# ShenhanQian/GaussianAvatars

Measured on NVIDIA H100. Metric: rasterizer fwd+bwd frames/sec @100k splats 1080p, higher is better.
Workload: dtype f32

## Files before the change

### gaussianavatars_b200/_native.py

```python
from __future__ import annotations

import ctypes as C
import os
import threading

import torch

_HERE = os.path.dirname(os.path.abspath(__file__))
LIB_PATH = os.path.join(_HERE, "libgaussianavatars_b200.so")

ABI_VERSION = 3
INPUT_ACTIVATED = 0
INPUT_BOUND_RAW = 1
SYNC_EXACT, SYNC_LATE, SYNC_NONE = 0, 1, 2
CTR_NOT_MIN_DEPTH_KEY, CTR_MAX_DEPTH_KEY, CTR_NUM_RENDERED, CTR_NUM_LISTED, CTR_BUCKET_OVERFLOW, CTR_CAPACITY, CTR_SEQ = range(7)
NUM_COUNTERS = 8
TUNE_HEAVY_FWD, TUNE_HEAVY_BWD, TUNE_DEPTH_SORT, TUNE_TILE_SORT, TUNE_NVLS_CTAS = 0, 1, 2, 4, 5

ALLOC_FN = C.CFUNCTYPE(C.c_void_p, C.c_void_p, C.c_size_t)


class ForwardArgs(C.Structure):
    _fields_ = [
        ("abi_version", C.c_uint32), ("input_mode", C.c_int32), ("P", C.c_int32), ("sh_degree", C.c_int32),
        ("sh_coeffs", C.c_int32), ("image_width", C.c_int32), ("image_height", C.c_int32),
        ("tanfovx", C.c_float), ("tanfovy", C.c_float), ("scale_modifier", C.c_float),
        ("prefiltered", C.c_int32), ("debug", C.c_int32), ("need_backward", C.c_int32), ("binning_hint", C.c_int32),
        ("exact_binning", C.c_int32), ("depth_hint_lo", C.c_uint32), ("depth_hint_hi", C.c_uint32),
        ("sync_mode", C.c_int32), ("frame_seq", C.c_uint32), ("counters_host", C.c_void_p),
        ("overflow_flag", C.c_void_p),
        ("bg", C.c_void_p), ("viewmatrix", C.c_void_p), ("projmatrix", C.c_void_p), ("campos", C.c_void_p),
        ("means3D", C.c_void_p), ("opacities", C.c_void_p), ("scales", C.c_void_p), ("rotations", C.c_void_p),
        ("cov3D_precomp", C.c_void_p), ("shs", C.c_void_p), ("sh_dc", C.c_void_p), ("sh_rest", C.c_void_p),
        ("colors_precomp", C.c_void_p),
        ("binding", C.c_void_p), ("num_faces", C.c_int32), ("face_center", C.c_void_p),
        ("face_orien_mat", C.c_void_p), ("face_scaling", C.c_void_p),
        ("out_color", C.c_void_p), ("radii", C.c_void_p), ("visibility", C.c_void_p),
        ("alloc_geom", ALLOC_FN), ("alloc_binning", ALLOC_FN), ("alloc_image", ALLOC_FN), ("alloc_user", C.c_void_p),
    ]


class FrameState(C.Structure):
    _fields_ = [
        ("num_rendered", C.c_int64), ("num_candidates", C.c_int64),
        ("geom_buffer", C.c_void_p), ("binning_buffer", C.c_void_p), ("image_buffer", C.c_void_p),
        ("geom_bytes", C.c_size_t), ("binning_bytes", C.c_size_t), ("image_bytes", C.c_size_t),
        ("sorted_selector", C.c_int32), ("sort_bits", C.c_int32), ("depth_bits", C.c_int32),
        ("depth_prefix", C.c_uint32), ("binning_capacity", C.c_int64),
        ("depth_key_min", C.c_uint32), ("depth_key_max", C.c_uint32), ("depth_sort_path", C.c_int32),
        ("attempts", C.c_int32), ("tile_sort_path", C.c_int32), ("reserved0", C.c_int32),
# ... 461 lines not shown
```

### gaussianavatars_b200/csrc/api.cu

```cuda
#include <atomic>
#include <chrono>
#include <cstdio>
#include <cstdlib>
#include <cstring>
#include <mutex>
#include <vector>

#include "common.cuh"
#include "kernels.cuh"

namespace gab {
static std::atomic<int64_t> g_launches{0};
void count_launch() { g_launches.fetch_add(1, std::memory_order_relaxed); }

struct SortTempCache {
  int64_t n = -1;
  int bits = -1;
  size_t bytes = 0;
};
static thread_local SortTempCache t_sort_cache[2];
static size_t cached_sort_temp_bytes(int64_t N, int bits) {
  SortTempCache& c = t_sort_cache[bits == 32 ? 0 : 1];
  if (c.bits != bits || N > c.n) {
    const int64_t n_up = N + N / 2 + 1024;
// ... 169 lines not shown
  cudaEvent_t fork = nullptr, join = nullptr;
  bool ok() {
    if (side == nullptr) {
      if (cudaStreamCreateWithFlags(&side, cudaStreamNonBlocking) != cudaSuccess) return false;
      if (cudaEventCreateWithFlags(&fork, cudaEventDisableTiming) != cudaSuccess) return false;
      if (cudaEventCreateWithFlags(&join, cudaEventDisableTiming) != cudaSuccess) return false;
    }
    return true;
  }
};
static thread_local CounterBranch t_branch[64];
static CounterBranch* counter_branch() {
  int dev = 0;
  if (cudaGetDevice(&dev) != cudaSuccess || dev < 0 || dev >= 64) return nullptr;
  return t_branch[dev].ok() ? &t_branch[dev] : nullptr;
}

static int check_arch() {
  constexpr int MAX_DEV = 64;
  static std::atomic<int> cached[MAX_DEV];
  int dev = 0, major = 0, minor = 0;
  if (cudaGetDevice(&dev) != cudaSuccess) return -1;
  const bool slot = dev >= 0 && dev < MAX_DEV;
  int c = slot ? cached[dev].load(std::memory_order_relaxed) : 0;
  if (c != 0) return c;
  if (cudaDeviceGetAttribute(&major, cudaDevAttrComputeCapabilityMajor, dev) != cudaSuccess) return -1;
  if (cudaDeviceGetAttribute(&minor, cudaDevAttrComputeCapabilityMinor, dev) != cudaSuccess) return -1;
  c = (major == 9 && minor == 0) ? 1 : -1;
  if (slot) cached[dev].store(c, std::memory_order_relaxed);
  return c;
}

static std::atomic<int> g_tune[GAB200_NUM_TUNABLES];
static const int g_tune_default[GAB200_NUM_TUNABLES] = {32, 2048, 0, 0, 0, 0, 0, 0};
int tune_get(int knob) {
  const int v = g_tune[knob].load(std::memory_order_relaxed);
  return v > 0 ? v - 1 : g_tune_default[knob];
}

static bool validate(const gab200_forward_args* a, bool display_only = false) {
  if (a == nullptr || a->abi_version != GAB200_ABI_VERSION) return false;
  if (a->P < 0 || a->image_width <= 0 || a->image_height <= 0) return false;
  if ((a->out_color == nullptr && !display_only) || (a->P > 0 && a->radii == nullptr)) return false;
  if (!a->bg || !a->viewmatrix || !a->projmatrix || !a->campos) return false;
  if (!a->alloc_geom || !a->alloc_binning || !a->alloc_image) return false;
  if (a->P == 0) return true;
  if (!a->means3D || !a->opacities) return false;
  if (a->sh_degree < 0 || a->sh_degree > 3) return false;
  const int nb = (a->sh_degree + 1) * (a->sh_degree + 1);
  if (a->input_mode == GAB200_INPUT_ACTIVATED) {
    const bool has_sr = a->scales != nullptr && a->rotations != nullptr;
    if (has_sr == (a->cov3D_precomp != nullptr)) return false;
    if ((a->scales != nullptr) != (a->rotations != nullptr)) return false;
    if ((a->shs != nullptr) == (a->colors_precomp != nullptr)) return false;
    if (a->shs != nullptr && a->sh_coeffs < nb) return false;
  } else if (a->input_mode == GAB200_INPUT_BOUND_RAW) {
    if (!a->scales || !a->rotations || a->cov3D_precomp) return false;
    if (a->colors_precomp == nullptr) {
      if (!a->sh_dc || a->sh_coeffs < nb) return false;
      if (a->sh_coeffs > 1 && !a->sh_rest) return false;
    }
    if (a->binding != nullptr && (!a->face_center || !a->face_orien_mat || !a->face_scaling || a->num_faces <= 0))
      return false;
  } else {
    return false;
  }
  return true;
// ... 97 lines not shown
  bool counting = true;
  uint32_t scan_clamp = 0xffffffffu;
  bool da = false;
  float* out_alpha = nullptr;
  float* out_depth = nullptr;
};

int enqueue_geometry(Frame& f, bool bucket, bool run_preprocess, uint32_t capacity) {
  const gab200_forward_args* a = f.a;
  GeomView& g = f.g;
  cudaStream_t stream = f.stream;
  DepthBuckets& d = g.buckets;
  d.enabled = 0;
  if (bucket) {
    d.lo = a->depth_hint_lo;
    d.hi = a->depth_hint_hi;
    d.scale = (float)((double)d.nb / ((double)(d.hi - d.lo) + 1.0));
    d.enabled = 1;
  }
  const int tiles = f.tiles;
  if (run_preprocess) {
    GAB_CUDA(cudaMemsetAsync(d.counts, 0, g.bucket_clear_bytes, stream));
    if (f.counting) GAB_CUDA(cudaMemsetAsync(f.iv.tile_count, 0, sizeof(uint32_t) * (size_t)tiles, stream));
    StageScope sc(GAB200_STAGE_PREPROCESS, stream);
    launch_preprocess(*a, f.views, f.cameras, f.tanfov, g.rec, g.aux, g.tiles_touched, f.nb ? g.clamped : nullptr,
                      g.depth_keys[0], g.ids[0], g.buckets, f.counting ? f.iv.tile_count : nullptr, f.da, stream);
  }
  GAB_STAGE_CHECK(f.dbg, stream);
  if (f.counting && run_preprocess) {
    StageScope sc(GAB200_STAGE_TILE_RANGES, stream);
    f.scan_clamp = capacity > 0 ? capacity : 0xffffffffu;
    launch_tile_scan_order(tiles, f.iv.tile_count, f.scan_clamp, f.iv.ranges, f.iv.tile_cursor, f.iv.order,
                           f.iv.order_info, g.buckets.meta, tune_get(GAB200_TUNE_HEAVY_FWD),
                           tune_get(GAB200_TUNE_HEAVY_BWD), stream);
  }
  {
    StageScope sc(GAB200_STAGE_SCAN, stream);
    if (bucket) {
      launch_depth_bucket_sort(f.P, g.buckets, g.depth_keys[0], g.tiles_touched, g.depth_keys[1], g.ids[1], g.offsets,
                               capacity, a->frame_seq, a->sync_mode == GAB200_SYNC_NONE ? a->overflow_flag : nullptr,
                               stream);
      f.selA = 1;
      f.order_count = g.buckets.meta + GAB200_CTR_NUM_LISTED;
    } else {
      GAB_CUDA(run_sort(g.sortA_temp, g.sortA_temp_bytes, g.depth_keys[0], g.depth_keys[1], g.ids[0], g.ids[1], f.P, 32,
                        &f.selA, stream));
      if (!f.counting)
        GAB_CUDA(run_scan(g.scan_temp, g.scan_temp_bytes, g.ids[f.selA], g.tiles_touched, g.offsets, f.P, stream));
      f.order_count = nullptr;
    }
    if (!bucket)
      launch_publish_counters(g.buckets.meta, f.counting ? nullptr : g.offsets, f.P, capacity, a->frame_seq,
                              a->sync_mode == GAB200_SYNC_NONE ? a->overflow_flag : nullptr, stream);
  }
  GAB_STAGE_CHECK(f.dbg, stream);
  if (f.branch != nullptr) {
    GAB_CUDA(cudaEventRecord(f.branch->fork, stream));
    GAB_CUDA(cudaStreamWaitEvent(f.branch->side, f.branch->fork, 0));
    GAB_CUDA(cudaMemcpyAsync(f.ctr_host, g.buckets.meta, sizeof(uint32_t) * GAB200_NUM_COUNTERS,
                             cudaMemcpyDeviceToHost, f.branch->side));
    GAB_CUDA(cudaEventRecord(f.branch->join, f.branch->side));
  } else {
    GAB_CUDA(cudaMemcpyAsync(f.ctr_host, g.buckets.meta, sizeof(uint32_t) * GAB200_NUM_COUNTERS,
                             cudaMemcpyDeviceToHost, stream));
  }
  if (f.ctr_event) GAB_CUDA(cudaEventRecord(f.ctr_event, stream));
  return GAB200_OK;
}

void emit(const Frame& f, const uint32_t* offsets, uint32_t cap, uint32_t* cursor, const BinView& bv,
          const EmitClears& clr) {
  launch_emit_keys(f.P, f.gx, f.gy, f.g.rec, f.g.aux, f.g.ids[f.selA], offsets, f.order_count, f.g.buckets.meta, cap,
                   cursor, bv.keys[0], bv.vals[0], f.a->exact_binning, f.cameras != nullptr ? f.a->P : 0, clr, f.stream);
}

int enqueue_binning_blend(Frame& f, void* bin, int64_t cap, int64_t n_known, size_t sort_temp, bool redo) {
  const gab200_forward_args* a = f.a;
  gab200_frame_state* st = f.st;
  cudaStream_t stream = f.stream;
  const int tiles = f.tiles;
  BinView bv = carve_binning(bin, cap, f.nb, sort_temp);
  st->binning_capacity = cap;
  st->binning_buffer = bin;
  st->binning_bytes = bv.bytes;
  const int64_t n_sort = n_known >= 0 ? n_known : cap;
  const bool counting = f.counting && f.P > 0;
  st->tile_sort_path = counting ? 1 : 0;
  EmitClears clr;
  clr.mask = n_sort > 0 ? bv.strip_mask : nullptr;
  clr.n_mask = (uint32_t)n_sort;
  int selector = 0;
  if (counting) {
    if (redo) {
      StageScope sc(GAB200_STAGE_TILE_RANGES, stream);
      f.scan_clamp = (uint32_t)(cap < 0xffffffffll ? cap : 0xffffffffll);
      launch_tile_scan_order(tiles, f.iv.tile_count, f.scan_clamp, f.iv.ranges, f.iv.tile_cursor, f.iv.order,
                             f.iv.order_info, f.g.buckets.meta, tune_get(GAB200_TUNE_HEAVY_FWD),
                             tune_get(GAB200_TUNE_HEAVY_BWD), stream);
    }
    if (n_sort > 0) {
      {
        StageScope sc(GAB200_STAGE_EMIT_KEYS, stream);
        emit(f, nullptr, (uint32_t)cap, f.iv.tile_cursor, bv, clr);
      }
      GAB_STAGE_CHECK(f.dbg, stream);
      {
        StageScope sc(GAB200_STAGE_SORT, stream);
        launch_tile_sort(tiles, f.iv.ranges, f.iv.order, f.iv.order_info, bv.keys[0], bv.vals[0], f.g.ids[f.selA],
                         f.order_count, f.P, stream);
      }
      GAB_STAGE_CHECK(f.dbg, stream);
    }
  } else {
    if (n_sort == 0) GAB_CUDA(cudaMemsetAsync(f.iv.ranges, 0, sizeof(uint2) * ((size_t)tiles + 1), stream));
    if (n_sort > 0) {
      clr.ranges = f.iv.ranges;
      clr.n_ranges = (uint32_t)tiles + 1;
      clr.sentinel = n_known < 0;
      {
        StageScope sc(GAB200_STAGE_EMIT_KEYS, stream);
        emit(f, f.g.offsets, (uint32_t)cap, nullptr, bv, clr);
      }
      GAB_STAGE_CHECK(f.dbg, stream);
      {
        StageScope sc(GAB200_STAGE_SORT, stream);
        GAB_CUDA(run_sort(bv.sort_temp, bv.sort_temp_bytes, bv.keys[0], bv.keys[1], bv.vals[0], bv.vals[1], n_sort,
                          st->sort_bits, &selector, stream));
      }
      GAB_STAGE_CHECK(f.dbg, stream);
      {
        StageScope sc(GAB200_STAGE_TILE_RANGES, stream);
        launch_tile_ranges(n_sort, (uint32_t)tiles, bv.keys[selector], f.iv.ranges, stream);
      }
      GAB_STAGE_CHECK(f.dbg, stream);
    }
    StageScope sc(GAB200_STAGE_TILE_RANGES, stream);
    launch_tile_scan_order(tiles, nullptr, 0xffffffffu, f.iv.ranges, nullptr, f.iv.order, f.iv.order_info, nullptr,
                           tune_get(GAB200_TUNE_HEAVY_FWD), tune_get(GAB200_TUNE_HEAVY_BWD), stream);
  }
  st->sorted_selector = selector;
  {
    StageScope sc(GAB200_STAGE_BLEND_FWD, stream);
    launch_blend_forward(f.views, f.W, f.H, f.iv.ranges, f.iv.order, f.iv.order_info, bv.vals[selector], f.g.rec, a->bg,
                         a->out_color, f.iv.final_T, f.iv.n_contrib, bv.strip_mask, f.out_rgb8, f.out_alpha,
                         f.out_depth, stream);
  }
  GAB_STAGE_CHECK(f.dbg, stream);
  return GAB200_OK;
}

int wait_counters(Frame& f) {
  for (;;) {
    const cudaError_t q = cudaEventQuery(f.ctr_event);
    if (q == cudaSuccess) return GAB200_OK;
    if (q != cudaErrorNotReady) return GAB200_ERR_CUDA;
  }
}
}

static int64_t run_forward(const gab200_forward_args* a, const float* tanfov, uint8_t* out_rgb8,
                           gab200_frame_state* st, void* stream_, int views = 1, const float* cameras = nullptr,
                           bool da = false, float* out_alpha = nullptr, float* out_depth = nullptr) {
  cudaStream_t stream = (cudaStream_t)stream_;
  if (!validate(a, out_rgb8 != nullptr && a != nullptr && a->need_backward == 0) || st == nullptr)
    return GAB200_ERR_INVALID_ARGUMENT;
  if (check_arch() < 0) return GAB200_ERR_ARCH;
  memset(st, 0, sizeof(*st));
  Frame f;
  f.a = a; f.tanfov = tanfov; f.out_rgb8 = out_rgb8; f.st = st; f.stream = stream;
  f.P = a->P * views; f.W = a->image_width; f.H = a->image_height;
  f.gx = (f.W + GAB_TILE - 1) / GAB_TILE; f.gy = (f.H + GAB_TILE - 1) / GAB_TILE;
// ... 818 lines not shown
```

### gaussianavatars_b200/csrc/blend.cu

```cuda
#include <type_traits>

#include "common.cuh"
#include "kernels.cuh"

namespace gab {

#define LOG2E 1.4426950408889634f
#define ALPHA_MIN (1.0f / 255.0f)
#define FULLMASK 0xffffffffu
#define CONIC_UNSCALE_AC (-2.0f / LOG2E)
#define CONIC_UNSCALE_B (-1.0f / LOG2E)

__device__ __forceinline__ float ex2_approx(float x) {
  float y;
  asm("ex2.approx.ftz.f32 %0, %1;" : "=f"(y) : "f"(x));
  return y;
}
__device__ __forceinline__ float rcp_approx(float x) {
  float y;
  asm("rcp.approx.ftz.f32 %0, %1;" : "=f"(y) : "f"(x));
  return y;
}
__device__ __forceinline__ void cp_async16(void* smem_dst, const void* gmem_src) {
  const unsigned s = (unsigned)__cvta_generic_to_shared(smem_dst);
// ... 1 lines not shown
}
__device__ __forceinline__ void cp_async_commit() { asm volatile("cp.async.commit_group;" ::: "memory"); }
template <int N>
__device__ __forceinline__ void cp_async_wait() {
  asm volatile("cp.async.wait_group %0;" ::"n"(N) : "memory");
}
__device__ __forceinline__ void gather_rec(SplatRec* dst, const SplatRec* src) {
  cp_async16(&dst->q0, &src->q0);
  cp_async16(&dst->q1, &src->q1);
  cp_async16(&dst->q2, &src->q2);
}

__device__ __forceinline__ uint32_t smem_u32(const void* p) { return (uint32_t)__cvta_generic_to_shared(p); }
__device__ __forceinline__ void mbar_init(uint64_t* bar, uint32_t count) {
  asm volatile("mbarrier.init.shared::cta.b64 [%0], %1;" ::"r"(smem_u32(bar)), "r"(count) : "memory");
}
__device__ __forceinline__ void mbar_fence_init() { asm volatile("fence.mbarrier_init.release.cluster;" ::: "memory"); }
__device__ __forceinline__ void mbar_arrive_expect_tx(uint64_t* bar, uint32_t bytes) {
  asm volatile("mbarrier.arrive.expect_tx.shared::cta.b64 _, [%0], %1;" ::"r"(smem_u32(bar)), "r"(bytes) : "memory");
}
__device__ __forceinline__ void bulk_copy_g2s(void* smem_dst, const void* gmem_src, uint32_t bytes, uint64_t* bar) {
  asm volatile("cp.async.bulk.shared::cluster.global.mbarrier::complete_tx::bytes [%0], [%1], %2, [%3];" ::"r"(
                   smem_u32(smem_dst)),
               "l"(gmem_src), "r"(bytes), "r"(smem_u32(bar))
               : "memory");
}
__device__ __forceinline__ void mbar_wait(uint64_t* bar, uint32_t parity) {
  asm volatile(
      "{\n\t.reg .pred p;\n\tMBAR_WAIT:\n\tmbarrier.try_wait.parity.shared::cta.b64 p, [%0], %1;\n\t@p bra MBAR_DONE;\n\t"
      "bra MBAR_WAIT;\n\tMBAR_DONE:\n\t}" ::"r"(smem_u32(bar)),
      "r"(parity)
      : "memory");
}
#define GAB_FWD_DEPTH_CTAS 2
#define GAB_FWD_VIEWS_TRAIN_CTAS 3
#define GAB_BWD_DEPTH_CTAS 5
#define ID_RING 3

template <int NT>
struct GroupBarrier {
  int id;
  __device__ __forceinline__ void sync() const { asm volatile("bar.sync %0, %1;" ::"r"(id), "n"(NT) : "memory"); }
  __device__ __forceinline__ bool sync_and(bool pred) const {
    unsigned r;
    asm volatile(
        "{\n\t.reg .pred p, q;\n\tsetp.ne.u32 q, %1, 0;\n\tbar.red.and.pred p, %2, %3, q;\n\tselp.u32 %0, 1, 0, p;\n\t}"
        : "=r"(r)
        : "r"((unsigned)pred), "r"(id), "n"(NT)
        : "memory");
    return r != 0;
  }
};

template <int K>
struct BandGeom {
  int col, row0, half, band0;
  __device__ __forceinline__ explicit BandGeom(int tl) {
    const int w = tl >> 5, lane = tl & 31;
    half = w & 1;
    band0 = (w >> 1) * K;
    col = half * 8 + (lane & 7);
    row0 = band0 * 4 + (lane >> 3);
  }
  __device__ __forceinline__ int bit(int i) const { return 2 * (band0 + i) + half; }
};

// ... 111 lines not shown
  if (nchunks > 0) {
    wait_ids(0);
    if (tl < n) gather_rec(&buf0[tl], rec + ids_ring[mis + tl]);
  }
  cp_async_commit();

  for (int c = 0; c < nchunks; c++) {
    SplatRec* nxt = ((c + 1) & 1) ? buf1 : buf0;
    if (c + 1 < nchunks) {
      wait_ids(c + 1);
      const int p = (c + 1) * NT + tl;
      if (p < n) gather_rec(&nxt[tl], rec + ids_ring[((c + 1) % ID_RING) * RING_STRIDE + mis + tl]);
    }
    cp_async_commit();
    if (tl == 0 && c + 2 < nchunks) issue_ids(c + 2);
    cp_async_wait<1>();
    if (bar.sync_and(done == ALL)) {
      if (c + 2 < nchunks) wait_ids(c + 2);
      break;
    }
    const SplatRec* cur = (c & 1) ? buf1 : buf0;
    const int cnt = min(NT, n - c * NT);
    const uint32_t pos0 = (uint32_t)(c * NT);
    uint32_t lb[K];
#pragma unroll
    for (int i = 0; i < K; i++) lb[i] = 0;
    for (int gbase = 0; gbase < cnt; gbase += 32) {
      const int gend = min(32, cnt - gbase);
      const uint32_t live = __ballot_sync(FULLMASK, lane < gend && reaches_rect(cur[gbase + lane], rx0, rx1, ry0, ry1));
      const int nlive = __popc(live);
      __syncwarp();
      if ((live >> lane) & 1u) my_idx[__popc(live & ((1u << lane) - 1u))] = (uint8_t)lane;
      __syncwarp();
#pragma unroll 4
      for (int k = 0; k < nlive; k++) {
        const int jj = my_idx[k];
        const SplatRec* r = cur + gbase + jj;
        const float4 q0 = r->q0;
        const float4 q1 = r->q1;
        const float dx = q0.x - fx;
        const float tA = q0.z * dx;
#pragma unroll
        for (int i = 0; i < K; i++) {
          const float dy = q0.y - fy[i];
          const float pw = fmaf(q1.x * dy, dy, fmaf(q0.w, dy, tA) * dx);
          const float alpha = fminf(0.99f, q1.y * ex2_approx(pw));
          if (pw <= 0.f && alpha >= ALPHA_MIN && !((done >> i) & 1u)) {
            const float test_T = T[i] * (1.f - alpha);
            if (test_T < 0.0001f) {
              done |= 1u << i;
            } else {
              const float w = alpha * T[i];
              Cr[i] = fmaf(q1.z, w, Cr[i]);
              Cg[i] = fmaf(q1.w, w, Cg[i]);
              Cb[i] = fmaf(r->q2.x, w, Cb[i]);
              if (DA) D[i] = fmaf(r->q2.w, w, D[i]);
              T[i] = test_T;
              last[i] = pos0 + (uint32_t)(gbase + jj) + 1u;
              lb[i] |= 1u << jj;
            }
          }
        }
      }
      if (want_mask) {
        uint32_t wh = 0;
#pragma unroll
        for (int i = 0; i < K; i++) {
// ... 16 lines not shown
  const float bg0 = bg[0], bg1 = bg[1], bg2 = bg[2];
  const size_t HW = (size_t)H * W;
#pragma unroll
  for (int i = 0; i < K; i++) {
    const int y = pixy0 + 4 * i;
    if (pixx < W && y < H) {
      const size_t pix = (size_t)y * W + pixx;
      if (OUT & BLEND_OUT_FLOAT) {
        out_color[pix] = fmaf(T[i], bg0, Cr[i]);
        out_color[HW + pix] = fmaf(T[i], bg1, Cg[i]);
        out_color[2 * HW + pix] = fmaf(T[i], bg2, Cb[i]);
      }
      if (TRAIN && final_T != nullptr) {
        final_T[pix] = T[i];
        n_contrib[pix] = last[i];
      }
      if (DA) {
        if (out_alpha != nullptr) out_alpha[pix] = 1.0f - T[i];
        if (out_depth != nullptr) out_depth[pix] = D[i];
      }
    }
  }
  if (OUT & BLEND_OUT_U8) {
#pragma unroll
    for (int i = 0; i < K; i++)
      store_display(out_rgb8, W, H, pixx, pixy0 + 4 * i, lane, fmaf(T[i], bg0, Cr[i]), fmaf(T[i], bg1, Cg[i]),
                    fmaf(T[i], bg2, Cb[i]));
  }
}

template <int OUT, bool DA, bool VIEWS>
__global__ void __launch_bounds__(256, DA                                 ? GAB_FWD_DEPTH_CTAS
                                       : VIEWS && (OUT & BLEND_OUT_TRAIN) ? GAB_FWD_VIEWS_TRAIN_CTAS
                                                                          : 0) blend_forward_kernel(
    int W, int H, int gx, int tiles, int view_tiles, const uint2* __restrict__ ranges, const uint32_t* __restrict__ order,
    const uint32_t* __restrict__ order_info, const uint32_t* __restrict__ point_list, const SplatRec* __restrict__ rec,
    const float* __restrict__ bg, float* __restrict__ out_color, float* __restrict__ final_T,
    uint32_t* __restrict__ n_contrib, uint8_t* __restrict__ strip_mask, uint8_t* __restrict__ out_rgb8,
    float* __restrict__ out_alpha, float* __restrict__ out_depth) {
  __shared__ SplatRec buf[2][256];
  __shared__ uint32_t smask[256];
  __shared__ __align__(16) uint32_t ids_ring[4][ID_RING * (64 + 4)];
  __shared__ __align__(8) uint64_t mbar[4][ID_RING];
  pdl_wait();
  pdl_trigger();
  const int nh = (int)order_info[0];
  const int b = blockIdx.x, t = threadIdx.x;
  if (b < nh) {
    forward_tile<1, OUT, DA, VIEWS>((int)order[b], t, GroupBarrier<256>{0}, buf[0], buf[1], smask, &ids_ring[0][0],
                                    mbar[0], W, H, gx, view_tiles, ranges, point_list, rec, bg, out_color, final_T,
                                    n_contrib, strip_mask, out_rgb8, out_alpha, out_depth);
  } else {
    const int g = t >> 6, slot = nh + 4 * (b - nh) + g;
    if (slot >= tiles) return;
    forward_tile<4, OUT, DA, VIEWS>((int)order[slot], t & 63, GroupBarrier<64>{1 + g}, buf[0] + g * 64,
                                    buf[1] + g * 64, smask + g * 64, ids_ring[g], mbar[g], W, H, gx, view_tiles, ranges,
                                    point_list, rec, bg, out_color, final_T, n_contrib, strip_mask, out_rgb8,
                                    out_alpha, out_depth);
  }
}

template <bool DA, bool VIEWS>
static decltype(&blend_forward_kernel<BLEND_OUT_FLOAT, DA, VIEWS>) blend_forward_instance(int out) {
  constexpr int F = BLEND_OUT_FLOAT, U = BLEND_OUT_U8, T = BLEND_OUT_TRAIN;
  if constexpr (!DA) {
    if (out == (F | T)) return blend_forward_kernel<F | T, DA, VIEWS>;
    if (out == (F | U | T)) return blend_forward_kernel<F | U | T, DA, VIEWS>;
  }
  out &= F | U;
  return out == F ? blend_forward_kernel<F, DA, VIEWS>
         : out == U ? blend_forward_kernel<U, DA, VIEWS>
                    : blend_forward_kernel<F | U, DA, VIEWS>;
}

void launch_blend_forward(int views, int W, int H, const uint2* ranges, const uint32_t* order,
                          const uint32_t* order_info, const uint32_t* point_list, const SplatRec* rec, const float* bg,
                          float* out_color, float* final_T, uint32_t* n_contrib, uint8_t* strip_mask, uint8_t* out_rgb8,
                          float* out_alpha, float* out_depth, cudaStream_t stream) {
  const int gx = (W + GAB_TILE - 1) / GAB_TILE, gy = (H + GAB_TILE - 1) / GAB_TILE;
  const int view_tiles = gx * gy, tiles = views * view_tiles;
  if (tiles == 0) return;
  const int out = (out_color != nullptr ? BLEND_OUT_FLOAT : 0) | (out_rgb8 != nullptr ? BLEND_OUT_U8 : 0) |
                  (final_T != nullptr ? BLEND_OUT_TRAIN : 0);
  const bool da = out_alpha != nullptr || out_depth != nullptr;
  auto kernel = da ? (views > 1 ? blend_forward_instance<true, true>(out) : blend_forward_instance<true, false>(out))
                   : (views > 1 ? blend_forward_instance<false, true>(out) : blend_forward_instance<false, false>(out));
// ... 61 lines not shown
    p.ar[i] = fmaf(al, er, p.ar[i]);
    p.ag[i] = fmaf(al, eg, p.ag[i]);
    p.ab[i] = fmaf(al, eb, p.ab[i]);
    if constexpr (DA) p.az[i] = fmaf(al, ez, p.az[i]);
    const float t = Gv * dLda;
    s.go += t;
    const float s_ = op * t;
    const float sd = s_ * dy;
    s.S0 += s_;
    s.S1 += sd;
    s.S2 = fmaf(sd, dy, s.S2);
  }
}

template <int K, int I, bool DA = false>
struct BandLoop {
  static __device__ __forceinline__ void run(uint32_t m, PixStateT<K, DA>& p, int pos, float py, float tA, float dx,
                                             float Bp, float Cp, float op, float cr, float cg, float cb,
                                             SplatSumsT<DA>& s, float cz = 0.f) {
    if (m & (1u << I)) visit_bands<K, (1 << I), DA>(p, pos, py, tA, dx, Bp, Cp, op, cr, cg, cb, s, cz);
    BandLoop<K, I + 1, DA>::run(m, p, pos, py, tA, dx, Bp, Cp, op, cr, cg, cb, s, cz);
  }
};
template <int K, bool DA>
struct BandLoop<K, K, DA> {
  static __device__ __forceinline__ void run(uint32_t, PixStateT<K, DA>&, int, float, float, float, float, float, float,
                                             float, float, float, SplatSumsT<DA>&, float = 0.f) {}
};

#define ROWS_STRIDE 36
template <int NR>
struct __align__(16) WarpSmemT {
  SplatRec rec[2][32];
  float rows[2][NR * ROWS_STRIDE];
  float part[2][32];
  uint32_t ids[ID_RING][32 + 4];
  uint8_t masks[ID_RING][32 + 16];
  uint64_t mbar[ID_RING];
};

template <int K, bool DA>
__device__ __forceinline__ void backward_task(int tile, int tl, WarpSmemT<DA ? 10 : 9>& sm, int W, int H, int gx,
                                              const uint2* __restrict__ ranges,
                                              const uint32_t* __restrict__ point_list,
                                              const SplatRec* __restrict__ rec, const float* __restrict__ bg,
                                              const float* __restrict__ final_T,
                                              const uint32_t* __restrict__ n_contrib,
                                              const float* __restrict__ dL_dpix,
                                              const uint8_t* __restrict__ strip_mask, float* __restrict__ g2d,
                                              const float* __restrict__ dL_dalpha,
                                              const float* __restrict__ dL_ddepth) {
  constexpr int NR = DA ? 10 : 9;
  const int tx = tile % gx, ty = tile / gx;
  const int lane = tl & 31;
  const BandGeom<K> geo(tl);
  const int pixx = tx * GAB_TILE + geo.col;
  const int pixy0 = ty * GAB_TILE + geo.row0;
  const float fx = (float)pixx;
  const uint2 range = ranges[tile];
  const size_t HW = (size_t)H * W;
  const float bg0 = bg[0], bg1 = bg[1], bg2 = bg[2];

  PixStateT<K, DA> p;
  int n = 0;
#pragma unroll
  for (int i = 0; i < K; i++) {
    const int y = pixy0 + 4 * i;
    p.fy[i] = (float)y;
// ... 40 lines not shown
  __syncwarp();
  auto issue_lists = [&](int k) {
    const uint32_t lo = range.x + (uint32_t)chunk_lo(k);
    uint64_t* b = &sm.mbar[k % ID_RING];
    mbar_arrive_expect_tx(b, TX_BYTES);
    bulk_copy_g2s(sm.ids[k % ID_RING], point_list + (lo & ~3u), (32 + 4) * 4, b);
    bulk_copy_g2s(sm.masks[k % ID_RING], strip_mask + (lo & ~15u), 32 + 16, b);
  };
  const int bit0 = geo.bit(0);
  auto stage_chunk = [&](int k, uint32_t& id, uint32_t& mine) {
    mbar_wait(&sm.mbar[k % ID_RING], (uint32_t)((k / ID_RING) & 1));
    const int q = k * 32 + lane;
    id = 0xffffffffu;
    mine = 0u;
    if (q < n) {
      const int lo = chunk_lo(k);
      const uint32_t g0 = range.x + (uint32_t)lo;
      const int rel = (n - 1 - q) - lo;
      id = sm.ids[k % ID_RING][(int)(g0 & 3u) + rel];
      const uint32_t mask = sm.masks[k % ID_RING][(int)(g0 & 15u) + rel];
#pragma unroll
      for (int i = 0; i < K; i++) mine |= ((mask >> (bit0 + 2 * i)) & 1u) << i;
      if (mine) gather_rec(&sm.rec[k & 1][lane], rec + id);
    }
    cp_async_commit();
  };
  if (lane == 0) {
    issue_lists(0);
    if (nchunks > 1) issue_lists(1);
  }
  uint32_t id_c, mine_c, id_n = 0xffffffffu, mine_n = 0u;
  stage_chunk(0, id_c, mine_c);

  uint32_t id1 = 0xffffffffu, id2 = 0xffffffffu;
  uint32_t par = 0;
  const int c1 = min(lane >> 1, NR - 1), h1 = lane & 1;
  auto reduce_step = [&](uint32_t id_rows, uint32_t id_part) {
    const float2 pp = *reinterpret_cast<const float2*>(&sm.part[par][2 * min(lane, NR - 1)]);
    const float4* r4 = reinterpret_cast<const float4*>(&sm.rows[par ^ 1][c1 * ROWS_STRIDE + h1 * 16]);
    const float4 a = r4[0], b = r4[1], c = r4[2], d = r4[3];
    if (id_part != 0xffffffffu && lane < NR) atomicAdd(g2d + (size_t)id_part * GAB_G2D_STRIDE + lane, pp.x + pp.y);
    const float s = (((a.x + a.y) + (a.z + a.w)) + ((b.x + b.y) + (b.z + b.w))) +
                    (((c.x + c.y) + (c.z + c.w)) + ((d.x + d.y) + (d.z + d.w)));
    if (id_rows != 0xffffffffu && lane < 2 * NR) sm.part[par ^ 1][lane] = s;
  };

  for (int c = 0; c < nchunks; c++) {
    __syncwarp();
    if (c + 1 < nchunks) stage_chunk(c + 1, id_n, mine_n);
    else cp_async_commit();
    if (lane == 0 && c + 2 < nchunks) issue_lists(c + 2);
    cp_async_wait<1>();
    __syncwarp();
    const SplatRec* cur = sm.rec[c & 1];
    uint32_t todo = __ballot_sync(FULLMASK, mine_c != 0u);
    while (todo) {
      const int jj = __ffs(todo) - 1;
      todo &= todo - 1;
      const uint32_t m = __shfl_sync(FULLMASK, mine_c, jj);
      const uint32_t id0 = __shfl_sync(FULLMASK, id_c, jj);
      const int pos = n - 1 - (c * 32 + jj);
      __syncwarp();
      const float4 q0 = cur[jj].q0;
      const float4 q1 = cur[jj].q1;
      const float cbl = cur[jj].q2.x;
      const float czl = DA ? cur[jj].q2.w : 0.f;
      reduce_step(id1, id2);
      const float dx = q0.x - fx;
      const float tA = q0.z * dx;
      SplatSumsT<DA> s;
      s.S0 = s.S1 = s.S2 = s.go = s.gr = s.gg = s.gb = 0.f;
      if constexpr (DA) s.gz = 0.f;
      if (m == (1u << K) - 1u)
        visit_bands<K, (1 << K) - 1, DA>(p, pos, q0.y, tA, dx, q0.w, q1.x, q1.y, q1.z, q1.w, cbl, s, czl);
      else BandLoop<K, 0, DA>::run(m, p, pos, q0.y, tA, dx, q0.w, q1.x, q1.y, q1.z, q1.w, cbl, s, czl);
      const float A = q0.z * CONIC_UNSCALE_AC, B = q0.w * CONIC_UNSCALE_B, C = q1.x * CONIC_UNSCALE_AC;
      const float dxS0 = dx * s.S0;
      float* row = &sm.rows[par][lane];
      row[0 * ROWS_STRIDE] = (-A * dxS0 - B * s.S1) * half_W;
      row[1 * ROWS_STRIDE] = (-C * s.S1 - B * dxS0) * half_H;
      row[2 * ROWS_STRIDE] = -0.5f * dx * dxS0;
      row[3 * ROWS_STRIDE] = -0.5f * dx * s.S1;
      row[4 * ROWS_STRIDE] = -0.5f * s.S2;
      row[5 * ROWS_STRIDE] = s.go;
      row[6 * ROWS_STRIDE] = s.gr;
      row[7 * ROWS_STRIDE] = s.gg;
      row[8 * ROWS_STRIDE] = s.gb;
      if constexpr (DA) row[9 * ROWS_STRIDE] = s.gz;
      id2 = id1;
      id1 = id0;
      par ^= 1;
    }
    id_c = id_n;
    mine_c = mine_n;
  }
  cp_async_wait<0>();
#pragma unroll
  for (int k = 0; k < 2; k++) {
    __syncwarp();
    reduce_step(id1, id2);
    id2 = id1;
    id1 = 0xffffffffu;
    par ^= 1;
  }
}

template <bool DA, bool VIEWS>
__global__ void __launch_bounds__(128, DA ? GAB_BWD_DEPTH_CTAS : 5) blend_backward_kernel(
    int W, int H, int gx, int tiles, int view_tiles, const uint2* __restrict__ ranges,
    const uint32_t* __restrict__ order, const uint32_t* __restrict__ order_info, const uint32_t* __restrict__ point_list,
    const SplatRec* __restrict__ rec, const float* __restrict__ bg, const float* __restrict__ final_T,
    const uint32_t* __restrict__ n_contrib, const float* __restrict__ dL_dpix, const uint8_t* __restrict__ strip_mask,
    float* __restrict__ g2d, const float* __restrict__ dL_dalpha, const float* __restrict__ dL_ddepth) {
  __shared__ WarpSmemT<DA ? 10 : 9> sm[4];
  pdl_wait();
  pdl_trigger();
  const int nh = (int)order_info[1];
  const int b = blockIdx.x, t = threadIdx.x, w = t >> 5;
  const bool heavy = b < nh;
  const int slot = heavy ? b : nh + 2 * (b - nh) + (w >> 1);
  if (!heavy && slot >= tiles) return;
  const int tile = (int)order[slot];
  const int view = VIEWS ? tile / view_tiles : 0, local = tile - view * view_tiles;
  const size_t off = (size_t)view * H * W;
  const uint2* vr = ranges + (size_t)view * view_tiles;
  const float* va = dL_dalpha != nullptr ? dL_dalpha + off : nullptr;
  const float* vz = dL_ddepth != nullptr ? dL_ddepth + off : nullptr;
  if (heavy)
    backward_task<2, DA>(local, t, sm[w], W, H, gx, vr, point_list, rec, bg, final_T + off, n_contrib + off,
                         dL_dpix + 3 * off, strip_mask, g2d, va, vz);
  else
    backward_task<4, DA>(local, t & 63, sm[w], W, H, gx, vr, point_list, rec, bg, final_T + off, n_contrib + off,
                         dL_dpix + 3 * off, strip_mask, g2d, va, vz);
}

void launch_blend_backward(int views, int W, int H, const uint2* ranges, const uint32_t* order,
                           const uint32_t* order_info, const uint32_t* point_list, const SplatRec* rec, const float* bg,
// ... 14 lines not shown
```

### gaussianavatars_b200/csrc/kernels.cuh

```cuda
#pragma once
#include "common.cuh"

namespace gab {

#define SH_C0 0.28209479177387814f
#define SH_C1 0.4886025119029199f
#define SH_C2_0 1.0925484305920792f
#define SH_C2_1 -1.0925484305920792f
#define SH_C2_2 0.31539156525252005f
#define SH_C2_3 -1.0925484305920792f
#define SH_C2_4 0.5462742152960396f
#define SH_C3_0 -0.5900435899266435f
#define SH_C3_1 2.890611442640554f
#define SH_C3_2 -0.4570457994644658f
#define SH_C3_3 0.3731763325901154f
#define SH_C3_4 -0.4570457994644658f
#define SH_C3_5 1.445305721320277f
#define SH_C3_6 -0.5900435899266435f

void count_launch();
int tune_get(int knob);

template <typename... Params, typename... Args>
void launch_pdl(void (*kernel)(Params...), dim3 grid, dim3 block, size_t smem, cudaStream_t stream, Args&&... args) {
// ... 66 lines not shown
  if (key >= d.hi) return d.nb - 1u;
  const uint32_t b = (uint32_t)(__uint2float_rz(key - d.lo) * d.scale);
  return b < d.nb ? b : d.nb - 1u;
}
void launch_preprocess(const gab200_forward_args& a, int views, const float* cameras, const float* tanfov,
                       SplatRec* rec, SplatAux* aux, uint32_t* tiles_touched, uint8_t* clamped, uint32_t* depth_keys,
                       uint32_t* ids, const DepthBuckets& buckets, uint32_t* tile_count, bool rec_depth,
                       cudaStream_t stream);
void launch_depth_bucket_sort(int P, const DepthBuckets& buckets, const uint32_t* depth_keys,
                              const uint32_t* tiles_touched, uint32_t* scratch_keys, uint32_t* sorted_ids,
                              uint32_t* offsets, uint32_t capacity, uint32_t seq, uint32_t* sticky_overflow,
                              cudaStream_t stream);
void launch_bind_activate(const gab200_forward_args& a, float* means3D, float* opacities, float* scales, float* cov3D,
                          cudaStream_t stream);
void launch_mark_visible(int P, const float* means3D, const float* V, uint8_t* present, cudaStream_t stream);
void launch_publish_counters(uint32_t* counters, const uint32_t* offsets, int P, uint32_t capacity, uint32_t seq,
                             uint32_t* sticky_overflow, cudaStream_t stream);
struct EmitClears {
  bool sentinel = false;
  uint8_t* mask = nullptr;
  uint32_t n_mask = 0;
  uint2* ranges = nullptr;
  uint32_t n_ranges = 0;
};
void launch_emit_keys(int P, int gx, int gy, const SplatRec* rec, const SplatAux* aux, const uint32_t* order,
                      const uint32_t* offsets, const uint32_t* order_count, const uint32_t* counters, uint32_t capacity,
                      uint32_t* cursor, uint32_t* keys, uint32_t* vals, int exact_binning, int view_splats,
                      const EmitClears& clr, cudaStream_t stream);
void launch_tile_ranges(int64_t N, uint32_t tiles, const uint32_t* keys, uint2* ranges, cudaStream_t stream);
void launch_expand_keys(int64_t N, const uint32_t* tile_keys, const uint32_t* ids, const SplatAux* aux, uint64_t* out,
                        cudaStream_t stream);
#define GAB_TILE_SORT_SMEM 2048
void launch_tile_scan_order(int tiles, const uint32_t* tile_count, uint32_t clamp, uint2* ranges, uint32_t* cursor,
                            uint32_t* order, uint32_t* order_info, uint32_t* counters, int heavy_fwd, int heavy_bwd,
                            cudaStream_t stream);
void launch_tile_sort(int tiles, const uint2* ranges, const uint32_t* order, const uint32_t* order_info, uint32_t* keys,
                      uint32_t* vals, const uint32_t* rank_to_id, const uint32_t* listed, int P, cudaStream_t stream);
void launch_expand_keys_by_range(int tiles, const uint2* ranges, const uint32_t* ids, const SplatAux* aux, uint64_t* out,
                                 cudaStream_t stream);

size_t scan_temp_bytes(int P);
cudaError_t run_scan(void* temp, size_t temp_bytes, const uint32_t* order, const uint32_t* tiles_touched, uint32_t* out,
                     int P, cudaStream_t stream);
size_t sort_temp_bytes(int64_t N, int end_bit);
cudaError_t run_sort(void* temp, size_t temp_bytes, uint32_t* keys_a, uint32_t* keys_b, uint32_t* vals_a,
                     uint32_t* vals_b, int64_t N, int end_bit, int* selector_out, cudaStream_t stream);

void launch_blend_forward(int views, int W, int H, const uint2* ranges, const uint32_t* order,
                          const uint32_t* order_info, const uint32_t* point_list, const SplatRec* rec, const float* bg,
                          float* out_color, float* final_T, uint32_t* n_contrib, uint8_t* strip_mask, uint8_t* out_rgb8,
                          float* out_alpha, float* out_depth, cudaStream_t stream);
void launch_blend_backward(int views, int W, int H, const uint2* ranges, const uint32_t* order,
                           const uint32_t* order_info, const uint32_t* point_list, const SplatRec* rec, const float* bg,
                           const float* final_T, const uint32_t* n_contrib, const float* dL_dpix,
                           const uint8_t* strip_mask, float* g2d, bool da, const float* dL_dalpha,
                           const float* dL_ddepth, cudaStream_t stream);
void launch_preprocess_backward(const gab200_backward_args& b, int views, const float* cameras, const float* tanfov,
                                const SplatAux* aux, const uint8_t* clamped, const float* g2d, float* face_scratch,
                                bool da, cudaStream_t stream);
#define GAB_FACE_GRAD_STRIDE 13

void launch_face_frame_forward(int F, const float* verts, const int32_t* faces, float* fc, float* fR, float* fs,
                               cudaStream_t stream);
void launch_face_frame_backward(int F, const float* verts, const int32_t* faces, const float* g_fc, const float* g_fR,
                                const float* g_fs, float* g_verts, cudaStream_t stream);

void launch_l1_loss_u8(int64_t n, const float* img, const uint8_t* gt, const float* upstream, float* grad, float* loss,
                       cudaStream_t stream);
// ... 87 lines not shown
```

### gaussianavatars_b200/csrc/tile_sort.cu

```cuda
#include "common.cuh"
#include "kernels.cuh"

namespace gab {

#define ORDER_NB 64
#define ORDER_WARPS 32
#define SCAN_NT 1024
#define ORDER_UNROLL 8

__global__ void __launch_bounds__(SCAN_NT) tile_scan_order_kernel(int tiles, const uint32_t* __restrict__ tile_count,
                                                                   uint32_t clamp, uint2* __restrict__ ranges,
                                                                   uint32_t* __restrict__ cursor,
                                                                   uint32_t* __restrict__ order,
                                                                   uint32_t* __restrict__ order_info,
                                                                   uint32_t* __restrict__ counters, int heavy_fwd,
                                                                   int heavy_bwd) {
  __shared__ uint32_t warp_tot[SCAN_NT / 32];
  __shared__ uint32_t s_carry;
  __shared__ uint32_t hist[ORDER_WARPS][ORDER_NB + 1];
  __shared__ uint32_t bucket_base[ORDER_NB];
  __shared__ uint32_t s_long;
  const int tid = threadIdx.x, lane = tid & 31, warp = tid >> 5;
  auto bucket = [](uint32_t len) -> int {
    return len == 0 ? ORDER_NB - 1 : (ORDER_NB - 2) - (int)min((uint32_t)(ORDER_NB - 2), len >> 5);
  };
  for (int k = tid; k < ORDER_WARPS * (ORDER_NB + 1); k += SCAN_NT) (&hist[0][0])[k] = 0;
  if (tid == 0) { s_carry = 0; s_long = 0; }
  __syncthreads();
  pdl_wait();
  pdl_trigger();
  if (tile_count != nullptr) {
    for (int base = 0; base < tiles; base += SCAN_NT) {
      const int t = base + tid;
      const uint32_t c = t < tiles ? tile_count[t] : 0u;
      uint32_t incl = c;
#pragma unroll
      for (int d = 1; d < 32; d <<= 1) {
        const uint32_t up = __shfl_up_sync(0xffffffffu, incl, d);
        if (lane >= d) incl += up;
      }
      if (lane == 31) warp_tot[warp] = incl;
      __syncthreads();
      uint32_t wbase = s_carry;
      for (int w = 0; w < warp; w++) wbase += warp_tot[w];
      const uint32_t start = wbase + incl - c;
      if (t < tiles) {
        ranges[t] = make_uint2(min(start, clamp), min(start + c, clamp));
        cursor[t] = start;
        atomicAdd(&hist[warp][bucket(min(start + c, clamp) - min(start, clamp))], 1u);
// ... 3 lines not shown
      if (tid == SCAN_NT - 1) s_carry = wbase + incl;
      __syncthreads();
    }
    if (tid == 0) counters[GAB200_CTR_NUM_RENDERED] = s_carry;
  } else {
    for (int base = 0; base < tiles; base += ORDER_UNROLL * SCAN_NT) {
      uint32_t len[ORDER_UNROLL];
#pragma unroll
      for (int k = 0; k < ORDER_UNROLL; k++) {
        const int t = base + k * SCAN_NT + tid;
        len[k] = 0xffffffffu;
        if (t < tiles) {
          const uint2 r = ranges[t];
          len[k] = r.y - r.x;
        }
      }
#pragma unroll
      for (int k = 0; k < ORDER_UNROLL; k++)
        if (base + k * SCAN_NT + tid < tiles) atomicAdd(&hist[warp][bucket(len[k])], 1u);
    }
    __syncthreads();
  }
  if (tid < ORDER_NB) {
    uint32_t run = 0;
    for (int w = 0; w < ORDER_WARPS; w++) {
      const uint32_t c = hist[w][tid];
      hist[w][tid] = run;
      run += c;
    }
    bucket_base[tid] = run;
  }
  __syncthreads();
  if (tid == 0) {
    uint32_t run = 0;
    const int qf = min(ORDER_NB - 2, max(1, heavy_fwd >> 5)), qb = min(ORDER_NB - 2, max(1, heavy_bwd >> 5));
    for (int b = 0; b < ORDER_NB; b++) {
      const uint32_t c = bucket_base[b];
      bucket_base[b] = run;
      run += c;
      if (b == (ORDER_NB - 2) - qf) order_info[0] = run;
      if (b == (ORDER_NB - 2) - qb) order_info[1] = run;
      if (b == 0) order_info[2] = s_long ? c : 0u;
    }
  }
  __syncthreads();
  for (int base = 0; base < tiles; base += ORDER_UNROLL * SCAN_NT) {
    uint32_t len[ORDER_UNROLL];
#pragma unroll
    for (int k = 0; k < ORDER_UNROLL; k++) {
      const int t = base + k * SCAN_NT + tid;
      len[k] = 0u;
      if (t < tiles) {
        const uint2 r = ranges[t];
        len[k] = r.y - r.x;
      }
    }
#pragma unroll
    for (int k = 0; k < ORDER_UNROLL; k++) {
      const int t = base + k * SCAN_NT + tid;
      if (t < tiles) {
        const int b = bucket(len[k]);
        order[bucket_base[b] + atomicAdd(&hist[warp][b], 1u)] = (uint32_t)t;
      }
    }
  }
}

void launch_tile_scan_order(int tiles, const uint32_t* tile_count, uint32_t clamp, uint2* ranges, uint32_t* cursor,
                            uint32_t* order, uint32_t* order_info, uint32_t* counters, int heavy_fwd, int heavy_bwd,
                            cudaStream_t stream) {
  if (tiles == 0) return;
  launch_pdl(tile_scan_order_kernel, 1, SCAN_NT, 0, stream, tiles, tile_count, clamp, ranges, cursor, order, order_info,
             counters, heavy_fwd, heavy_bwd);
}

#define TS_NT 128
__global__ void __launch_bounds__(TS_NT) tile_sort_kernel(int tiles, const uint2* __restrict__ ranges,
                                                          const uint32_t* __restrict__ order,
                                                          uint32_t* __restrict__ keys, uint32_t* __restrict__ vals) {
  __shared__ uint32_t sk[GAB_TILE_SORT_SMEM];
  __shared__ uint32_t sv[GAB_TILE_SORT_SMEM];
  const int tile = (int)order[blockIdx.x];
  const uint2 r = ranges[tile];
  const int n = (int)(r.y - r.x);
  if (n <= 1 || n > GAB_TILE_SORT_SMEM) return;
  const int tid = threadIdx.x;
  uint32_t* k = keys + r.x;
  uint32_t* v = vals + r.x;
  if (n <= 32) {
    if (tid >= 32) return;
    const uint32_t key = tid < n ? k[tid] : 0xffffffffu;
    const uint32_t val = tid < n ? v[tid] : 0u;
    int rank = 0;
#pragma unroll 8
    for (int j = 0; j < 32; j++) rank += __shfl_sync(0xffffffffu, key, j) < key ? 1 : 0;
    if (tid < n) v[rank] = val;
    return;
  }
  int m = 64;
  while (m < n) m <<= 1;
  for (int i = tid; i < m; i += TS_NT) {
    sk[i] = i < n ? k[i] : 0xffffffffu;
    sv[i] = i < n ? v[i] : 0u;
  }
  __syncthreads();
  for (int size = 2; size <= m; size <<= 1) {
// ... 118 lines not shown
```

### include/gab200_rasterizer.h

```cpp
#ifndef GAB200_RASTERIZER_H
#define GAB200_RASTERIZER_H

#include <stddef.h>
#include <stdint.h>

#ifdef __cplusplus
extern "C" {
#endif

#define GAB200_ABI_VERSION 3

typedef enum gab200_status {
  GAB200_OK = 0,
  GAB200_ERR_INVALID_ARGUMENT = -1,
  GAB200_ERR_CUDA = -2,
  GAB200_ERR_ALLOC = -3,
  GAB200_ERR_ARCH = -4,
  GAB200_ERR_OVERFLOW = -5
} gab200_status;

typedef enum gab200_input_mode {
  GAB200_INPUT_ACTIVATED = 0,
  GAB200_INPUT_BOUND_RAW = 1
} gab200_input_mode;
// ... 442 lines not shown
typedef struct gab200_flame_grads {
  float* expr;
  float* rotation;
  float* neck_pose;
  float* jaw_pose;
  float* eyes_pose;
  float* translation;
} gab200_flame_grads;
int32_t gab200_flame_backward(const gab200_flame_frame_args* args, const float* dL_dverts, const float* dL_dverts_cano,
                              const gab200_flame_grads* grads, void* stream);

int32_t gab200_export_binning(const gab200_forward_args* args, const gab200_frame_state* state, uint64_t* keys,
                              uint32_t* values, uint32_t* ranges, void* stream);

enum {
  GAB200_STAGE_PREPROCESS = 0,
  GAB200_STAGE_SCAN = 1,
  GAB200_STAGE_EMIT_KEYS = 2,
  GAB200_STAGE_SORT = 3,
  GAB200_STAGE_TILE_RANGES = 4,
  GAB200_STAGE_BLEND_FWD = 5,
  GAB200_STAGE_BLEND_BWD = 6,
  GAB200_STAGE_PREPROCESS_BWD = 7,
  GAB200_NUM_STAGES = 8
};
void gab200_stage_timing_enable(int32_t enable);
void gab200_host_times(double out[6], int32_t reset);
int32_t gab200_stage_times(double total_ms[GAB200_NUM_STAGES], int64_t launches[GAB200_NUM_STAGES], int32_t reset);

enum {
  GAB200_TUNE_HEAVY_FWD = 0,
  GAB200_TUNE_HEAVY_BWD = 1,
  GAB200_TUNE_DEPTH_SORT = 2,
  GAB200_TUNE_TILE_SORT = 4,
  GAB200_TUNE_NVLS_CTAS = 5,
  GAB200_NUM_TUNABLES = 8
};
int32_t gab200_tune(int32_t knob, int32_t value);

int64_t gab200_launch_count(void);

const char* gab200_status_string(int32_t status);
uint32_t gab200_abi_version(void);

#ifdef __cplusplus
}
#endif
#endif
```

Measured before the change: 1882.

## Add mid-tier two-tiles-per-CTA forward blend path with separate heavy threshold

```diff
diff --git a/gaussianavatars_b200/_native.py b/gaussianavatars_b200/_native.py
--- a/gaussianavatars_b200/_native.py
+++ b/gaussianavatars_b200/_native.py
@@ -15,7 +15,7 @@
 SYNC_EXACT, SYNC_LATE, SYNC_NONE = 0, 1, 2
 CTR_NOT_MIN_DEPTH_KEY, CTR_MAX_DEPTH_KEY, CTR_NUM_RENDERED, CTR_NUM_LISTED, CTR_BUCKET_OVERFLOW, CTR_CAPACITY, CTR_SEQ = range(7)
 NUM_COUNTERS = 8
-TUNE_HEAVY_FWD, TUNE_HEAVY_BWD, TUNE_DEPTH_SORT, TUNE_TILE_SORT, TUNE_NVLS_CTAS = 0, 1, 2, 4, 5
+TUNE_HEAVY_FWD, TUNE_HEAVY_BWD, TUNE_DEPTH_SORT, TUNE_MID_FWD, TUNE_TILE_SORT, TUNE_NVLS_CTAS = 0, 1, 2, 3, 4, 5
 
 ALLOC_FN = C.CFUNCTYPE(C.c_void_p, C.c_void_p, C.c_size_t)
 
diff --git a/gaussianavatars_b200/csrc/api.cu b/gaussianavatars_b200/csrc/api.cu
--- a/gaussianavatars_b200/csrc/api.cu
+++ b/gaussianavatars_b200/csrc/api.cu
@@ -225,7 +225,7 @@
 }
 
 static std::atomic<int> g_tune[GAB200_NUM_TUNABLES];
-static const int g_tune_default[GAB200_NUM_TUNABLES] = {32, 2048, 0, 0, 0, 0, 0, 0};
+static const int g_tune_default[GAB200_NUM_TUNABLES] = {2048, 2048, 0, 32, 0, 0, 0, 0};
 int tune_get(int knob) {
   const int v = g_tune[knob].load(std::memory_order_relaxed);
   return v > 0 ? v - 1 : g_tune_default[knob];
@@ -389,7 +389,7 @@
     f.scan_clamp = capacity > 0 ? capacity : 0xffffffffu;
     launch_tile_scan_order(tiles, f.iv.tile_count, f.scan_clamp, f.iv.ranges, f.iv.tile_cursor, f.iv.order,
                            f.iv.order_info, g.buckets.meta, tune_get(GAB200_TUNE_HEAVY_FWD),
-                           tune_get(GAB200_TUNE_HEAVY_BWD), stream);
+                           tune_get(GAB200_TUNE_MID_FWD), tune_get(GAB200_TUNE_HEAVY_BWD), stream);
   }
   {
     StageScope sc(GAB200_STAGE_SCAN, stream);
@@ -453,7 +453,7 @@
       f.scan_clamp = (uint32_t)(cap < 0xffffffffll ? cap : 0xffffffffll);
       launch_tile_scan_order(tiles, f.iv.tile_count, f.scan_clamp, f.iv.ranges, f.iv.tile_cursor, f.iv.order,
                              f.iv.order_info, f.g.buckets.meta, tune_get(GAB200_TUNE_HEAVY_FWD),
-                             tune_get(GAB200_TUNE_HEAVY_BWD), stream);
+                             tune_get(GAB200_TUNE_MID_FWD), tune_get(GAB200_TUNE_HEAVY_BWD), stream);
     }
     if (n_sort > 0) {
       {
@@ -493,7 +493,8 @@
     }
     StageScope sc(GAB200_STAGE_TILE_RANGES, stream);
     launch_tile_scan_order(tiles, nullptr, 0xffffffffu, f.iv.ranges, nullptr, f.iv.order, f.iv.order_info, nullptr,
-                           tune_get(GAB200_TUNE_HEAVY_FWD), tune_get(GAB200_TUNE_HEAVY_BWD), stream);
+                           tune_get(GAB200_TUNE_HEAVY_FWD), tune_get(GAB200_TUNE_MID_FWD), tune_get(GAB200_TUNE_HEAVY_BWD),
+                           stream);
   }
   st->sorted_selector = selector;
   {
diff --git a/gaussianavatars_b200/csrc/blend.cu b/gaussianavatars_b200/csrc/blend.cu
--- a/gaussianavatars_b200/csrc/blend.cu
+++ b/gaussianavatars_b200/csrc/blend.cu
@@ -57,6 +57,7 @@
       "r"(parity)
       : "memory");
 }
+#define GAB_FWD_CTAS 4
 #define GAB_FWD_DEPTH_CTAS 2
 #define GAB_FWD_VIEWS_TRAIN_CTAS 3
 #define GAB_BWD_DEPTH_CTAS 5
@@ -234,7 +235,7 @@
       __syncwarp();
       if ((live >> lane) & 1u) my_idx[__popc(live & ((1u << lane) - 1u))] = (uint8_t)lane;
       __syncwarp();
-#pragma unroll 4
+#pragma unroll (K == 1 ? 1 : 4)
       for (int k = 0; k < nlive; k++) {
         const int jj = my_idx[k];
         const SplatRec* r = cur + gbase + jj;
@@ -317,7 +318,7 @@
 template <int OUT, bool DA, bool VIEWS>
 __global__ void __launch_bounds__(256, DA                                 ? GAB_FWD_DEPTH_CTAS
                                        : VIEWS && (OUT & BLEND_OUT_TRAIN) ? GAB_FWD_VIEWS_TRAIN_CTAS
-                                                                          : 0) blend_forward_kernel(
+                                                                          : GAB_FWD_CTAS) blend_forward_kernel(
     int W, int H, int gx, int tiles, int view_tiles, const uint2* __restrict__ ranges, const uint32_t* __restrict__ order,
     const uint32_t* __restrict__ order_info, const uint32_t* __restrict__ point_list, const SplatRec* __restrict__ rec,
     const float* __restrict__ bg, float* __restrict__ out_color, float* __restrict__ final_T,
@@ -329,14 +330,22 @@
   __shared__ __align__(8) uint64_t mbar[4][ID_RING];
   pdl_wait();
   pdl_trigger();
-  const int nh = (int)order_info[0];
+  const int nd = (int)order_info[0], nm = (int)order_info[3];
+  const int bl = nd + (nm - nd + 1) / 2;
   const int b = blockIdx.x, t = threadIdx.x;
-  if (b < nh) {
+  if (b < nd) {
     forward_tile<1, OUT, DA, VIEWS>((int)order[b], t, GroupBarrier<256>{0}, buf[0], buf[1], smask, &ids_ring[0][0],
                                     mbar[0], W, H, gx, view_tiles, ranges, point_list, rec, bg, out_color, final_T,
                                     n_contrib, strip_mask, out_rgb8, out_alpha, out_depth);
+  } else if (b < bl) {
+    const int g = t >> 7, slot = nd + 2 * (b - nd) + g;
+    if (slot >= nm) return;
+    forward_tile<2, OUT, DA, VIEWS>((int)order[slot], t & 127, GroupBarrier<128>{1 + g}, buf[0] + g * 128,
+                                    buf[1] + g * 128, smask + g * 128, ids_ring[2 * g], mbar[g], W, H, gx, view_tiles,
+                                    ranges, point_list, rec, bg, out_color, final_T, n_contrib, strip_mask, out_rgb8,
+                                    out_alpha, out_depth);
   } else {
-    const int g = t >> 6, slot = nh + 4 * (b - nh) + g;
+    const int g = t >> 6, slot = nm + 4 * (b - bl) + g;
     if (slot >= tiles) return;
     forward_tile<4, OUT, DA, VIEWS>((int)order[slot], t & 63, GroupBarrier<64>{1 + g}, buf[0] + g * 64,
                                     buf[1] + g * 64, smask + g * 64, ids_ring[g], mbar[g], W, H, gx, view_tiles, ranges,
diff --git a/gaussianavatars_b200/csrc/kernels.cuh b/gaussianavatars_b200/csrc/kernels.cuh
--- a/gaussianavatars_b200/csrc/kernels.cuh
+++ b/gaussianavatars_b200/csrc/kernels.cuh
@@ -122,8 +122,8 @@
                         cudaStream_t stream);
 #define GAB_TILE_SORT_SMEM 2048
 void launch_tile_scan_order(int tiles, const uint32_t* tile_count, uint32_t clamp, uint2* ranges, uint32_t* cursor,
-                            uint32_t* order, uint32_t* order_info, uint32_t* counters, int heavy_fwd, int heavy_bwd,
-                            cudaStream_t stream);
+                            uint32_t* order, uint32_t* order_info, uint32_t* counters, int heavy_fwd, int mid_fwd,
+                            int heavy_bwd, cudaStream_t stream);
 void launch_tile_sort(int tiles, const uint2* ranges, const uint32_t* order, const uint32_t* order_info, uint32_t* keys,
                       uint32_t* vals, const uint32_t* rank_to_id, const uint32_t* listed, int P, cudaStream_t stream);
 void launch_expand_keys_by_range(int tiles, const uint2* ranges, const uint32_t* ids, const SplatAux* aux, uint64_t* out,
diff --git a/gaussianavatars_b200/csrc/tile_sort.cu b/gaussianavatars_b200/csrc/tile_sort.cu
--- a/gaussianavatars_b200/csrc/tile_sort.cu
+++ b/gaussianavatars_b200/csrc/tile_sort.cu
@@ -14,7 +14,7 @@
                                                                    uint32_t* __restrict__ order,
                                                                    uint32_t* __restrict__ order_info,
                                                                    uint32_t* __restrict__ counters, int heavy_fwd,
-                                                                   int heavy_bwd) {
+                                                                   int mid_fwd, int heavy_bwd) {
   __shared__ uint32_t warp_tot[SCAN_NT / 32];
   __shared__ uint32_t s_carry;
   __shared__ uint32_t hist[ORDER_WARPS][ORDER_NB + 1];
@@ -84,16 +84,20 @@
   }
   __syncthreads();
   if (tid == 0) {
-    uint32_t run = 0;
+    uint32_t run = 0, n_deep = 0, n_mid = 0;
     const int qf = min(ORDER_NB - 2, max(1, heavy_fwd >> 5)), qb = min(ORDER_NB - 2, max(1, heavy_bwd >> 5));
+    const int qm = min(ORDER_NB - 2, max(0, mid_fwd >> 5));
     for (int b = 0; b < ORDER_NB; b++) {
       const uint32_t c = bucket_base[b];
       bucket_base[b] = run;
       run += c;
-      if (b == (ORDER_NB - 2) - qf) order_info[0] = run;
+      if (b == (ORDER_NB - 2) - qf) n_deep = run;
+      if (b == (ORDER_NB - 2) - qm) n_mid = run;
       if (b == (ORDER_NB - 2) - qb) order_info[1] = run;
       if (b == 0) order_info[2] = s_long ? c : 0u;
     }
+    order_info[0] = n_deep;
+    order_info[3] = max(n_deep, n_mid);
   }
   __syncthreads();
   for (int base = 0; base < tiles; base += ORDER_UNROLL * SCAN_NT) {
@@ -119,11 +123,11 @@
 }
 
 void launch_tile_scan_order(int tiles, const uint32_t* tile_count, uint32_t clamp, uint2* ranges, uint32_t* cursor,
-                            uint32_t* order, uint32_t* order_info, uint32_t* counters, int heavy_fwd, int heavy_bwd,
-                            cudaStream_t stream) {
+                            uint32_t* order, uint32_t* order_info, uint32_t* counters, int heavy_fwd, int mid_fwd,
+                            int heavy_bwd, cudaStream_t stream) {
   if (tiles == 0) return;
   launch_pdl(tile_scan_order_kernel, 1, SCAN_NT, 0, stream, tiles, tile_count, clamp, ranges, cursor, order, order_info,
-             counters, heavy_fwd, heavy_bwd);
+             counters, heavy_fwd, mid_fwd, heavy_bwd);
 }
 
 #define TS_NT 128
diff --git a/include/gab200_rasterizer.h b/include/gab200_rasterizer.h
--- a/include/gab200_rasterizer.h
+++ b/include/gab200_rasterizer.h
@@ -498,6 +498,7 @@
   GAB200_TUNE_HEAVY_FWD = 0,
   GAB200_TUNE_HEAVY_BWD = 1,
   GAB200_TUNE_DEPTH_SORT = 2,
+  GAB200_TUNE_MID_FWD = 3,
   GAB200_TUNE_TILE_SORT = 4,
   GAB200_TUNE_NVLS_CTAS = 5,
   GAB200_NUM_TUNABLES = 8
```

Result: no change. 1911, median of 6 (+1.6%).

## Batch per-splat gradient row reductions three at a time in backward blend

Applied to the files above, without the earlier changes.

```diff
diff --git a/gaussianavatars_b200/csrc/blend.cu b/gaussianavatars_b200/csrc/blend.cu
--- a/gaussianavatars_b200/csrc/blend.cu
+++ b/gaussianavatars_b200/csrc/blend.cu
@@ -464,8 +464,7 @@
 template <int NR>
 struct __align__(16) WarpSmemT {
   SplatRec rec[2][32];
-  float rows[2][NR * ROWS_STRIDE];
-  float part[2][32];
+  float rows[3 * NR][ROWS_STRIDE];
   uint32_t ids[ID_RING][32 + 4];
   uint8_t masks[ID_RING][32 + 16];
   uint64_t mbar[ID_RING];
@@ -572,17 +571,21 @@
   uint32_t id_c, mine_c, id_n = 0xffffffffu, mine_n = 0u;
   stage_chunk(0, id_c, mine_c);
 
-  uint32_t id1 = 0xffffffffu, id2 = 0xffffffffu;
-  uint32_t par = 0;
-  const int c1 = min(lane >> 1, NR - 1), h1 = lane & 1;
-  auto reduce_step = [&](uint32_t id_rows, uint32_t id_part) {
-    const float2 pp = *reinterpret_cast<const float2*>(&sm.part[par][2 * min(lane, NR - 1)]);
-    const float4* r4 = reinterpret_cast<const float4*>(&sm.rows[par ^ 1][c1 * ROWS_STRIDE + h1 * 16]);
-    const float4 a = r4[0], b = r4[1], c = r4[2], d = r4[3];
-    if (id_part != 0xffffffffu && lane < NR) atomicAdd(g2d + (size_t)id_part * GAB_G2D_STRIDE + lane, pp.x + pp.y);
-    const float s = (((a.x + a.y) + (a.z + a.w)) + ((b.x + b.y) + (b.z + b.w))) +
-                    (((c.x + c.y) + (c.z + c.w)) + ((d.x + d.y) + (d.z + d.w)));
-    if (id_rows != 0xffffffffu && lane < 2 * NR) sm.part[par ^ 1][lane] = s;
+  int fill = 0;
+  const int my_slot = lane / NR;
+  uint32_t my_id = 0xffffffffu;
+  const float4* my_row = reinterpret_cast<const float4*>(sm.rows[min(lane, 3 * NR - 1)]);
+  float* my_g2d = g2d + lane % NR;
+  auto send_batch = [&]() {
+    __syncwarp();
+    float h[2];
+#pragma unroll
+    for (int k = 0; k < 2; k++) {
+      const float4 a = my_row[4 * k], b = my_row[4 * k + 1], c = my_row[4 * k + 2], d = my_row[4 * k + 3];
+      h[k] = (((a.x + a.y) + (a.z + a.w)) + ((b.x + b.y) + (b.z + b.w))) +
+             (((c.x + c.y) + (c.z + c.w)) + ((d.x + d.y) + (d.z + d.w)));
+    }
+    if (my_slot < fill) atomicAdd(my_g2d + (size_t)my_id * GAB_G2D_STRIDE, h[0] + h[1]);
   };
 
   for (int c = 0; c < nchunks; c++) {
@@ -605,7 +608,6 @@
       const float4 q1 = cur[jj].q1;
       const float cbl = cur[jj].q2.x;
       const float czl = DA ? cur[jj].q2.w : 0.f;
-      reduce_step(id1, id2);
       const float dx = q0.x - fx;
       const float tA = q0.z * dx;
       SplatSumsT<DA> s;
@@ -616,7 +618,7 @@
       else BandLoop<K, 0, DA>::run(m, p, pos, q0.y, tA, dx, q0.w, q1.x, q1.y, q1.z, q1.w, cbl, s, czl);
       const float A = q0.z * CONIC_UNSCALE_AC, B = q0.w * CONIC_UNSCALE_B, C = q1.x * CONIC_UNSCALE_AC;
       const float dxS0 = dx * s.S0;
-      float* row = &sm.rows[par][lane];
+      float* row = &sm.rows[fill * NR][lane];
       row[0 * ROWS_STRIDE] = (-A * dxS0 - B * s.S1) * half_W;
       row[1 * ROWS_STRIDE] = (-C * s.S1 - B * dxS0) * half_H;
       row[2 * ROWS_STRIDE] = -0.5f * dx * dxS0;
@@ -627,22 +629,17 @@
       row[7 * ROWS_STRIDE] = s.gg;
       row[8 * ROWS_STRIDE] = s.gb;
       if constexpr (DA) row[9 * ROWS_STRIDE] = s.gz;
-      id2 = id1;
-      id1 = id0;
-      par ^= 1;
+      if (my_slot == fill) my_id = id0;
+      if (++fill == 3) {
+        send_batch();
+        fill = 0;
+      }
     }
     id_c = id_n;
     mine_c = mine_n;
   }
   cp_async_wait<0>();
-#pragma unroll
-  for (int k = 0; k < 2; k++) {
-    __syncwarp();
-    reduce_step(id1, id2);
-    id2 = id1;
-    id1 = 0xffffffffu;
-    par ^= 1;
-  }
+  if (fill > 0) send_batch();
 }
 
 template <bool DA, bool VIEWS>
```

Result: faster. 1875 before, 1952 after (median of 6 runs) (+4.1%).
